# joelle-o-world/dusp

Hardware: AMD Instinct MI355X
Metric: rendered Msamples/sec (whole node) + HBM GB/s fraction, 1024-voice 48kHz (higher is better)
Workload: dtype f64; 1 GPU; configs[2] per-voice: 1024 voices/GPU x Multiply(Osc(10k), Ramp(T,1,0) triggered), 60s @48000 Hz, every voice's PCM written; voices_per_gpu=1024, voices_total=1024, n_samples=2880000, engine=fused, parallelism=voices sharded over 1 GPU(s), no collective

## Files before the change

dusp_amd/csrc/modmath.hpp:

```cpp
#pragma once
#if !defined(__HIPCC_RTC__)
#include <cstdint>
#endif

#if !defined(DUSP_HOST_DEVICE)
#if defined(__HIPCC__)
#define DUSP_HOST_DEVICE __host__ __device__ __forceinline__
#else
#define DUSP_HOST_DEVICE inline
#endif
#endif

namespace dusp {
namespace {

DUSP_HOST_DEVICE uint64_t addmod(uint64_t a, uint64_t b, uint64_t S) {
    const uint64_t s = a + b;
    return s >= S ? s - S : s;
}
DUSP_HOST_DEVICE uint64_t mulmod(uint64_t a, uint64_t n, uint64_t S) {
    uint64_t acc = 0;
    for (int bit = 63 - __builtin_clzll(n | 1); bit >= 0; --bit) {
        acc = addmod(acc, acc, S);
        if ((n >> bit) & 1) acc = addmod(acc, a, S);
    }
    return acc;
}

DUSP_HOST_DEVICE uint32_t mod_u32(uint32_t x, uint32_t m, double inv_m) {
    const uint32_t q = (uint32_t)((double)x * inv_m);
    uint32_t r = x - q * m;
    if ((int32_t)r < 0) r += m;
    if (r >= m) r -= m;
    return r;
}
DUSP_HOST_DEVICE uint64_t mod_u64(uint64_t x, uint64_t m, double inv_m) {
    const uint64_t q = (uint64_t)((double)x * inv_m);
    uint64_t r = x - q * m;
    if ((int64_t)r < 0) r += m;
    if ((int64_t)r < 0) r += m;
    if (r >= m) r -= m;
    if (r >= m) r -= m;
    return r;
}

DUSP_HOST_DEVICE unsigned long long jit_mulmod(unsigned long long a, unsigned long long n, unsigned long long S, double inv_S) {
    const unsigned long long ah = a >> 32, al = a & 0xffffffffull;
    unsigned long long r = mod_u64(ah * n, S, inv_S);
    r = mod_u64(r << 11, S, inv_S);
    r = mod_u64(r << 11, S, inv_S);
    r = mod_u64(r << 10, S, inv_S);
    return addmod(r, mod_u64(al * n, S, inv_S), S);
}

DUSP_HOST_DEVICE uint64_t sum_block_base(uint64_t B0, uint64_t bs, uint64_t bs256, uint32_t blk, uint64_t S, double inv_S) {
    return mod_u64(B0 + (uint64_t)(blk >> 8) * bs256 + (uint64_t)(blk & 255u) * bs, S, inv_S);
}
DUSP_HOST_DEVICE uint32_t sum_block_base_int(uint32_t B0, uint32_t bs, uint32_t blk, uint32_t sr, double inv_sr) {
    return mod_u32(B0 + blk * bs, sr, inv_sr);
}
DUSP_HOST_DEVICE bool sum_int_blocks_ok(uint32_t n_blocks, uint32_t sr) { return ((uint64_t)n_blocks + 1) * sr < (1ull << 32); }

}
}
```

dusp_amd/csrc/sumchain_engine.hip:

```cpp
#include <hip/hip_runtime.h>

#include "device_types.hpp"
#include "fused_device.hpp"
#include "fused_plan.hpp"

namespace dusp {

template <int TBL, bool INT, int GB, bool FINITE, int BLOCK, int ENV>
__global__ void __launch_bounds__(BLOCK) dusp_sumchain_kernel(SumArgs A) {
    extern __shared__ __attribute__((aligned(16))) float lds_table[];
    Table<TBL> table;
    table.g = A.table;
    table.h = lds_table;
    table.N = A.sample_rate + 1;
    table.M = A.sample_rate / 2;
    if (TBL == 1) load_half_table<BLOCK>(lds_table, A.table, A.sample_rate);

    const uint32_t lane = threadIdx.x & 63u;
    constexpr uint32_t waves_per_block = BLOCK / 64;
    const uint64_t n_items = (uint64_t)A.n_inst * A.n_blocks;
    const uint64_t total_waves = (uint64_t)gridDim.x * waves_per_block;
    const uint32_t sr = A.sample_rate;
    const uint32_t n_full = A.vec4_ok ? (uint32_t)(A.n_samples / kChunk) : 0u;

    for (uint64_t item = (uint64_t)blockIdx.x * waves_per_block + (threadIdx.x >> 6); item < n_items; item += total_waves) {
        const uint32_t blk = (uint32_t)(item % A.n_blocks);
        const uint32_t inst = (uint32_t)(item / A.n_blocks);
        const uint32_t g0 = blk * GB;
        const size_t row_at = (size_t)inst * A.n_samples + (size_t)g0 * kChunk + lane * 4;
        float acc[GB][4];
#pragma unroll
        for (int g = 0; g < GB; ++g)
            for (int c = 0; c < 4; ++c) acc[g][c] = 0.f;
        if (A.init) {
#pragma unroll
            for (int g = 0; g < GB; ++g)
                if (g0 + g < n_full) {
                    const f32x4 v = *(const f32x4 *)(A.init + row_at + (size_t)g * kChunk);
                    acc[g][0] = v[0]; acc[g][1] = v[1]; acc[g][2] = v[2]; acc[g][3] = v[3];
                } else if (g0 + g < A.n_groups) {
                    const uint64_t t = (uint64_t)(g0 + g) * kChunk + lane * 4;
                    for (int c = 0; c < 4; ++c)
                        if (t + c < A.n_samples) acc[g][c] = A.init[row_at + (size_t)g * kChunk + c];
                }
        }
        float env[ENV == 2 ? GB : 1][4];
        if (ENV == 2) {
            const double dy = A.r_y1 - A.r_y0, rcp = 1.0 / A.r_d;
#pragma unroll
            for (int g = 0; g < (ENV == 2 ? GB : 1); ++g)
#pragma unroll
                for (int c = 0; c < 4; ++c) {
                    const uint64_t n = A.first + (uint64_t)(g0 + g) * kChunk + lane * 4 + c;
                    const double tt = A.r_playing ? fmin(A.r_t0 + (double)(n + 1), A.r_d) : A.r_t0;
                    double q;
                    if (A.r_fastdiv) {
                        q = tt * rcp;
                        q = fma(fma(-q, A.r_d, tt), rcp, q);
                    } else
                        q = tt / A.r_d;
                    env[g][c] = (float)(A.r_y0 + q * dy);
                }
        }

        for (uint32_t j = 0; j < A.n_voices; ++j) {
            const SumVoice rc = A.voices[j];
            if (INT) {
                const uint32_t f = (uint32_t)(rc.Fm >> 32), s4 = (uint32_t)(rc.step4 >> 32), s256 = (uint32_t)(rc.step256 >> 32);
                const uint32_t base = sum_block_base_int((uint32_t)(rc.B0 >> 32), (uint32_t)(rc.bs >> 32), blk, sr, A.inv_sr);
                uint32_t idx[4];
                idx[0] = mod_u32(base + lane * s4, sr, A.inv_sr);
#pragma unroll
                for (int c = 1; c < 4; ++c) {
                    idx[c] = idx[c - 1] + f;
                    idx[c] = min(idx[c], idx[c] - sr);
                }
#pragma unroll
                for (int g = 0; g < GB; ++g)
#pragma unroll
                    for (int c = 0; c < 4; ++c) {
                        float v = table.at(idx[c]);
                        if (ENV == 1) v = v * rc.gain;
                        if (ENV == 2) v = v * env[g][c];
                        acc[g][c] = acc[g][c] + v;
                        idx[c] += s256;
                        idx[c] = min(idx[c], idx[c] - sr);
                    }
            } else {
                const uint64_t base = sum_block_base(rc.B0, rc.bs, A.bs256[j], blk, A.S, A.inv_S);
                uint64_t P = mod_u64(base + (uint64_t)lane * rc.step4, A.S, A.inv_S);
                uint32_t I[4], F[4];
#pragma unroll
                for (int c = 0; c < 4; ++c) {
                    I[c] = (uint32_t)(P >> 32);
                    F[c] = (uint32_t)P;
                    P += rc.Fm;
                    if (P >= A.S) P -= A.S;
                }
                const uint32_t dI = (uint32_t)(rc.step256 >> 32), dF = (uint32_t)rc.step256;
#pragma unroll
                for (int g = 0; g < GB; ++g)
#pragma unroll
                    for (int c = 0; c < 4; ++c) {
                        float ta, tb;
                        table.pair(I[c], ta, tb);
                        const double wb = (double)F[c];
                        const double wa = 4294967296.0 - wb;
                        const float x = (float)((double)ta * wa + (double)tb * wb);
                        float v = ldexpf(x, -32);
                        if (ENV == 1) v = v * rc.gain;
                        if (ENV == 2) v = v * env[g][c];
                        acc[g][c] = acc[g][c] + v;
                        const uint32_t f2 = F[c] + dF;
                        uint32_t i2 = I[c] + dI + (f2 < F[c] ? 1u : 0u);
                        i2 = min(i2, i2 - sr);
                        F[c] = f2;
                        I[c] = i2;
                    }
            }
        }
        float *row = A.out + row_at;
#pragma unroll
        for (int g = 0; g < GB; ++g) {
            const uint32_t gg = g0 + g;
            if (gg >= A.n_groups) break;
            float v[4];
            for (int c = 0; c < 4; ++c) v[c] = A.raw ? acc[g][c] : fix_out<FINITE>(acc[g][c]);
            if (gg < n_full)
                store4<true>(row, v, 0, A.n_samples);
            else
                store4<false>(row, v, (uint64_t)gg * kChunk + lane * 4, A.n_samples);
            row += kChunk;
        }
    }
}

template <int TBL, bool INT, int GB, bool FINITE, int BLOCK, int ENV>
static hipError_t launch_sum(const SumArgs &A, int grid, size_t lds_bytes, hipStream_t stream) {
    auto kernel = dusp_sumchain_kernel<TBL, INT, GB, FINITE, BLOCK, ENV>;
    if (lds_bytes > 65536) {
        hipError_t e = hipFuncSetAttribute((const void *)kernel, hipFuncAttributeMaxDynamicSharedMemorySize, (int)lds_bytes);
        if (e != hipSuccess) return e;
    }
    hipLaunchKernelGGL(kernel, dim3((unsigned)grid), dim3(BLOCK), lds_bytes, stream, A);
    return hipGetLastError();
}

hipError_t launch_sumchain(const FusedPlan &plan, const FusedLaunch &L, const SumVoice *d_voices, int gb, hipStream_t stream) {
    SumArgs A{};
    A.voices = d_voices;
    A.bs256 = (const uint64_t *)(d_voices + plan.sum_f.size());
    A.table = L.tables + (size_t)plan.table_id * L.table_stride;
    A.out = L.out;
    A.n_samples = L.n_samples;
    A.S = (uint64_t)L.sample_rate << 32;
    A.inv_S = 1.0 / (double)A.S;
    A.inv_sr = 1.0 / (double)L.sample_rate;
    A.n_voices = (uint32_t)plan.sum_f.size();
    A.n_inst = L.n_inst;
    A.first = L.chain_first;
    A.init = L.chain_init;
    A.raw = L.chain_raw ? 1u : 0u;
    const uint32_t window_groups = (uint32_t)((L.n_samples + kChunk - 1) / kChunk);
    A.n_groups = window_groups;
    A.n_blocks = (window_groups + gb - 1) / gb;
    A.sample_rate = L.sample_rate;
    A.vec4_ok = (L.n_samples % 4 == 0) && (((uintptr_t)L.out & 15) == 0);
    A.r_d = plan.r_d;
    A.r_y0 = plan.r_y0;
    A.r_y1 = plan.r_y1;
    A.r_t0 = plan.r_t0;
    A.r_playing = plan.r_playing;
    A.r_fastdiv = plan.r_fastdiv;

    const bool tbl = L.table_antisym && L.sample_rate % 2 == 0 && half_table_lds_bytes(L.sample_rate) <= 160 * 1024;
    const size_t lds_bytes = tbl ? half_table_lds_bytes(L.sample_rate) : 0;
    const int grid = tbl ? L.n_cus : L.n_cus * 8;
    const bool finite = L.table_finite && plan.sum_env == 0;
    const bool use_int = plan.sum_all_int && sum_int_blocks_ok(A.n_blocks, L.sample_rate);

#define DUSP_S5(TB, IN, G, FIN, EN) \
    return TB ? launch_sum<1, IN, G, FIN, 1024, EN>(A, grid, lds_bytes, stream) : launch_sum<0, IN, G, FIN, 256, EN>(A, grid, 0, stream)
#define DUSP_S4(TB, IN, G, FIN) \
    do { if (plan.sum_env == 2) { DUSP_S5(TB, IN, G, FIN, 2); } if (plan.sum_env == 1) { DUSP_S5(TB, IN, G, FIN, 1); } DUSP_S5(TB, IN, G, FIN, 0); } while (0)
#define DUSP_S3(IN, G) \
    do { if (finite) { DUSP_S4(tbl, IN, G, true); } DUSP_S4(tbl, IN, G, false); } while (0)
    if (gb == 8) {
        if (use_int) DUSP_S3(true, 8);
        DUSP_S3(false, 8);
    }
    if (use_int) DUSP_S3(true, 4);
    DUSP_S3(false, 4);
#undef DUSP_S3
#undef DUSP_S4
#undef DUSP_S5
}

}
```

Baseline: 1.553 million Msamples/s.

## Reshape LDS half-table addressing and prefetch voice params in sum-chain kernel

Replaces the floating-point modulo with a multiply-high magic-number reduction, and prefetches the next voice's parameters into scalar registers via readfirstlane. In the integer path with an LDS table, it keeps phase indices scaled by four and looks up the antisymmetric half table with a v_sad_u32 mirror plus a padded byte address, so each lookup needs fewer instructions. Loads are batched in groups of four behind a scheduling barrier so LDS latency overlaps. It also changes the wave-to-item mapping and lets excess blocks exit early. The inline asm depends on a hand-computed LDS base and padding layout, which risks addressing mistakes and adds a little LDS.

```diff
diff --git a/dusp_amd/csrc/modmath.hpp b/dusp_amd/csrc/modmath.hpp
--- a/dusp_amd/csrc/modmath.hpp
+++ b/dusp_amd/csrc/modmath.hpp
@@ -60,6 +60,20 @@
     return mod_u32(B0 + blk * bs, sr, inv_sr);
 }
 DUSP_HOST_DEVICE bool sum_int_blocks_ok(uint32_t n_blocks, uint32_t sr) { return ((uint64_t)n_blocks + 1) * sr < (1ull << 32); }
+DUSP_HOST_DEVICE uint32_t mod_u32_magic(uint32_t sr) { return 0xffffffffu / sr; }
+DUSP_HOST_DEVICE uint32_t mod_u32_mulhi(uint32_t x, uint32_t sr, uint32_t magic) {
+    const uint32_t q = (uint32_t)(((uint64_t)x * magic) >> 32);
+    const uint32_t r = x - q * sr;
+    return r < r - sr ? r : r - sr;
+}
+DUSP_HOST_DEVICE uint32_t sum_block_base_int_mulhi(uint32_t B0, uint32_t bs, uint32_t blk, uint32_t sr, uint32_t magic) {
+    return mod_u32_mulhi(B0 + blk * bs, sr, magic);
+}
+DUSP_HOST_DEVICE uint32_t half_image_k4(uint32_t i4, uint32_t M) { return (i4 > 4u * M + 2u ? i4 - (4u * M + 2u) : 4u * M + 2u - i4) + 2u; }
+DUSP_HOST_DEVICE uint32_t half_image_byte(uint32_t k4) { return k4 + ((k4 >> 7) << 2); }
+constexpr uint32_t kHalfImageSlack = 144;
+DUSP_HOST_DEVICE uint32_t half_image_bias(uint32_t lds_base) { return (((lds_base * 32u + 32u) / 33u) + 127u) & ~127u; }
+DUSP_HOST_DEVICE uint32_t half_image_start(uint32_t bias) { return bias + (bias >> 5); }
 
 }
 }
diff --git a/dusp_amd/csrc/sumchain_engine.hip b/dusp_amd/csrc/sumchain_engine.hip
--- a/dusp_amd/csrc/sumchain_engine.hip
+++ b/dusp_amd/csrc/sumchain_engine.hip
@@ -6,24 +6,75 @@
 
 namespace dusp {
 
+struct VoiceFetch {
+    SumVoice rc;
+    uint64_t bs256;
+};
+__device__ __forceinline__ uint64_t high_word_of(const uint64_t *p) { return (uint64_t)((const uint32_t *)p)[1] << 32; }
+template <bool INT, int ENV>
+__device__ __forceinline__ VoiceFetch fetch_voice(const SumArgs &A, uint32_t j) {
+    const SumVoice *p = A.voices + j;
+    VoiceFetch v;
+    v.rc.B0 = INT ? high_word_of(&p->B0) : p->B0;
+    v.rc.bs = INT ? high_word_of(&p->bs) : p->bs;
+    v.rc.step4 = INT ? high_word_of(&p->step4) : p->step4;
+    v.rc.step256 = INT ? high_word_of(&p->step256) : p->step256;
+    v.rc.Fm = INT ? high_word_of(&p->Fm) : p->Fm;
+    v.rc.gain = ENV == 1 ? p->gain : 1.f;
+    v.rc.pad = 0;
+    v.bs256 = INT ? 0ull : A.bs256[j];
+    return v;
+}
+__device__ __forceinline__ uint32_t uniform32(uint32_t x) { return (uint32_t)__builtin_amdgcn_readfirstlane((int)x); }
+__device__ __forceinline__ uint64_t uniform64(uint64_t x) { return ((uint64_t)uniform32((uint32_t)(x >> 32)) << 32) | uniform32((uint32_t)x); }
+__device__ __forceinline__ VoiceFetch uniform_voice(const VoiceFetch &v) {
+    VoiceFetch u;
+    u.rc.B0 = uniform64(v.rc.B0);
+    u.rc.bs = uniform64(v.rc.bs);
+    u.rc.step4 = uniform64(v.rc.step4);
+    u.rc.step256 = uniform64(v.rc.step256);
+    u.rc.Fm = uniform64(v.rc.Fm);
+    u.rc.gain = __uint_as_float(uniform32(__float_as_uint(v.rc.gain)));
+    u.rc.pad = 0;
+    u.bs256 = uniform64(v.bs256);
+    return u;
+}
+
+typedef const __attribute__((address_space(3))) float *LdsFloatPtr;
+__device__ __forceinline__ float half_image_at4(uint32_t i4, uint32_t mid4_v, uint32_t bias2) {
+    uint32_t k4, at;
+    asm("v_sad_u32 %0, %1, %2, %3" : "=v"(k4) : "v"(i4), "v"(mid4_v), "s"(bias2));
+    asm("v_lshl_add_u32 %0, %1, 2, %2" : "=v"(at) : "v"(k4 >> 7), "v"(k4));
+    return *(LdsFloatPtr)(uintptr_t)at;
+}
+
 template <int TBL, bool INT, int GB, bool FINITE, int BLOCK, int ENV>
 __global__ void __launch_bounds__(BLOCK) dusp_sumchain_kernel(SumArgs A) {
     extern __shared__ __attribute__((aligned(16))) float lds_table[];
+    const uint64_t n_items = (uint64_t)A.n_inst * A.n_blocks;
+    if (blockIdx.x >= n_items) return;
     Table<TBL> table;
     table.g = A.table;
-    table.h = lds_table;
+    const uint32_t lds_base = (uint32_t)(uintptr_t)(LdsFloatPtr)lds_table, bias = half_image_bias(lds_base);
+    float *image = lds_table + (half_image_start(bias) - lds_base) / 4;
+    table.h = image;
     table.N = A.sample_rate + 1;
     table.M = A.sample_rate / 2;
-    if (TBL == 1) load_half_table<BLOCK>(lds_table, A.table, A.sample_rate);
+    if (TBL == 1) load_half_table<BLOCK>(image, A.table, A.sample_rate);
 
     const uint32_t lane = threadIdx.x & 63u;
+    const uint32_t wave = uniform32(threadIdx.x >> 6);
     constexpr uint32_t waves_per_block = BLOCK / 64;
-    const uint64_t n_items = (uint64_t)A.n_inst * A.n_blocks;
     const uint64_t total_waves = (uint64_t)gridDim.x * waves_per_block;
     const uint32_t sr = A.sample_rate;
     const uint32_t n_full = A.vec4_ok ? (uint32_t)(A.n_samples / kChunk) : 0u;
-
-    for (uint64_t item = (uint64_t)blockIdx.x * waves_per_block + (threadIdx.x >> 6); item < n_items; item += total_waves) {
+    const uint32_t magic = mod_u32_magic(sr);
+    constexpr uint32_t Q = (INT && TBL == 1) ? 4u : 1u;
+    const uint32_t srq = sr * Q, mid4 = 4u * (sr / 2) + 2u;
+    uint32_t mid4_v = mid4;
+    asm("" : "+v"(mid4_v));
+
+    for (uint64_t item = (uint64_t)wave * gridDim.x + blockIdx.x; item < n_items; item += total_waves) {
         const uint32_t blk = (uint32_t)(item % A.n_blocks);
         const uint32_t inst = (uint32_t)(item / A.n_blocks);
         const uint32_t g0 = blk * GB;
@@ -63,31 +114,49 @@
                 }
         }
 
+        VoiceFetch next{};
+        if (A.n_voices) next = fetch_voice<INT, ENV>(A, 0);
         for (uint32_t j = 0; j < A.n_voices; ++j) {
-            const SumVoice rc = A.voices[j];
+            const VoiceFetch cur = uniform_voice(next);
+            const SumVoice &rc = cur.rc;
+            next = fetch_voice<INT, ENV>(A, min(j + 1, A.n_voices - 1));
+            asm volatile("" ::: "memory");
             if (INT) {
-                const uint32_t f = (uint32_t)(rc.Fm >> 32), s4 = (uint32_t)(rc.step4 >> 32), s256 = (uint32_t)(rc.step256 >> 32);
-                const uint32_t base = sum_block_base_int((uint32_t)(rc.B0 >> 32), (uint32_t)(rc.bs >> 32), blk, sr, A.inv_sr);
+                const uint32_t f = (uint32_t)(rc.Fm >> 32) * Q, s4 = (uint32_t)(rc.step4 >> 32), s256 = (uint32_t)(rc.step256 >> 32) * Q;
+                const uint32_t base = sum_block_base_int_mulhi((uint32_t)(rc.B0 >> 32), (uint32_t)(rc.bs >> 32), blk, sr, magic);
                 uint32_t idx[4];
-                idx[0] = mod_u32(base + lane * s4, sr, A.inv_sr);
+                idx[0] = mod_u32_mulhi(base + lane * s4, sr, magic) * Q;
 #pragma unroll
                 for (int c = 1; c < 4; ++c) {
                     idx[c] = idx[c - 1] + f;
-                    idx[c] = min(idx[c], idx[c] - sr);
-                }
-#pragma unroll
-                for (int g = 0; g < GB; ++g)
-#pragma unroll
-                    for (int c = 0; c < 4; ++c) {
-                        float v = table.at(idx[c]);
-                        if (ENV == 1) v = v * rc.gain;
-                        if (ENV == 2) v = v * env[g][c];
-                        acc[g][c] = acc[g][c] + v;
-                        idx[c] += s256;
-                        idx[c] = min(idx[c], idx[c] - sr);
-                    }
+                    idx[c] = min(idx[c], idx[c] - srq);
+                }
+#pragma unroll
+                for (int h = 0; h < GB; h += 4) {
+                    float val[4][4];
+                    bool upper[4][4];
+#pragma unroll
+                    for (int g = 0; g < 4; ++g)
+#pragma unroll
+                        for (int c = 0; c < 4; ++c) {
+                            val[g][c] = Q == 4 ? half_image_at4(idx[c], mid4_v, bias + 2u) : table.at(idx[c]);
+                            upper[g][c] = Q == 4 && idx[c] > mid4;
+                            idx[c] += s256;
+                            idx[c] = min(idx[c], idx[c] - srq);
+                        }
+                    __builtin_amdgcn_sched_barrier(0);
+#pragma unroll
+                    for (int g = 0; g < 4; ++g)
+#pragma unroll
+                        for (int c = 0; c < 4; ++c) {
+                            float v = upper[g][c] ? -val[g][c] : val[g][c];
+                            if (ENV == 1) v = v * rc.gain;
+                            if (ENV == 2) v = v * env[h + g][c];
+                            acc[h + g][c] = acc[h + g][c] + v;
+                        }
+                }
             } else {
-                const uint64_t base = sum_block_base(rc.B0, rc.bs, A.bs256[j], blk, A.S, A.inv_S);
+                const uint64_t base = sum_block_base(rc.B0, rc.bs, cur.bs256, blk, A.S, A.inv_S);
                 uint64_t P = mod_u64(base + (uint64_t)lane * rc.step4, A.S, A.inv_S);
                 uint32_t I[4], F[4];
 #pragma unroll
@@ -173,8 +242,9 @@
     A.r_playing = plan.r_playing;
     A.r_fastdiv = plan.r_fastdiv;
 
-    const bool tbl = L.table_antisym && L.sample_rate % 2 == 0 && half_table_lds_bytes(L.sample_rate) <= 160 * 1024;
-    const size_t lds_bytes = tbl ? half_table_lds_bytes(L.sample_rate) : 0;
+    const size_t image_bytes = half_table_lds_bytes(L.sample_rate) + kHalfImageSlack;
+    const bool tbl = L.table_antisym && L.sample_rate % 2 == 0 && image_bytes <= 160 * 1024;
+    const size_t lds_bytes = tbl ? image_bytes : 0;
     const int grid = tbl ? L.n_cus : L.n_cus * 8;
     const bool finite = L.table_finite && plan.sum_env == 0;
     const bool use_int = plan.sum_all_int && sum_int_blocks_ok(A.n_blocks, L.sample_rate);
```

New measurement: 1.517 million Msamples/s. 0.977x the previous value.
